# Dave-he/unet-watermark

Hardware: AMD Instinct MI355X
Metric: train_images_per_sec (higher is better)
Workload: dtype f32 storage and accumulation; the convolution products of the encoder and decoder layers (3x3, 7x7 stem, stride-2 and 1x1 layers: forward, data gradients, and the weight gradients of the stride-1 3x3 layers and the stem) as fp16x3 splits - every fp32 operand = two fp16 halves (22 mantissa bits), a*b; 1 GPU; Unet-resnet34 512x512 bs16/GPU train step: fwd + Dice + bwd + Adam (BASELINE.json configs[1]); global_batch=16, parallelism=dp1, grad_allreduce=none

## Files before the change

include/uwm.h:

```cpp
#ifndef UWM_H
#define UWM_H
#include <stddef.h>
#include <stdint.h>

#ifdef __cplusplus
extern "C" {
#endif

typedef struct uwm_model* uwm_handle;
typedef void* uwm_stream;

enum { UWM_ENC_RESNET18 = 18, UWM_ENC_RESNET34 = 34, UWM_ENC_RESNET50 = 50,
       UWM_ENC_EFFICIENTNET_B0 = 100, UWM_ENC_EFFICIENTNET_B1 = 101, UWM_ENC_EFFICIENTNET_B2 = 102,
       UWM_ENC_EFFICIENTNET_B3 = 103, UWM_ENC_EFFICIENTNET_B4 = 104, UWM_ENC_EFFICIENTNET_B5 = 105,
       UWM_ENC_EFFICIENTNET_B6 = 106, UWM_ENC_EFFICIENTNET_B7 = 107 };
enum { UWM_ARCH_UNET = 0, UWM_ARCH_UNETPLUSPLUS = 1 };
enum { UWM_T_F32 = 0, UWM_T_I64 = 1, UWM_T_U8 = 2, UWM_T_I32 = 3 };
enum { UWM_KIND_CONV_W = 0, UWM_KIND_BIAS = 1, UWM_KIND_BN_GAMMA = 2, UWM_KIND_BN_BETA = 3,
       UWM_KIND_BN_MEAN = 4, UWM_KIND_BN_VAR = 5 };
enum { UWM_ARENA_PARAM = 0, UWM_ARENA_BUFFER = 1 };
enum { UWM_PREC_F32 = 0, UWM_PREC_BF16X3 = 1, UWM_PREC_BF16X3_ALL = 2, UWM_PREC_F16X3 = 3, UWM_PREC_F16X3_ALL = 4,
       UWM_PREC_F16X1 = 5, UWM_PREC_F16X3_BWD2 = 6 };

typedef struct {
// ... 356 lines not shown
int    uwm_op_morph(const uint8_t* in, uint8_t* out, int N, int H, int W, int dilate, int shape, int kw, int kh,
                    int iterations, void* workspace, size_t workspace_bytes, uwm_stream stream);
int    uwm_op_components(const uint8_t* in, int32_t* labels ,
                         int32_t* areas , int N, int H, int W,
                         void* workspace, size_t workspace_bytes, uwm_stream stream);

int  uwm_set_side_stream(uwm_handle h, int on);

int  uwm_prof_enable(int on);
int  uwm_prof_collect(double* out, int max_classes);
const char* uwm_prof_class_name(int cls);

int  uwm_debug_lookup(uwm_handle h, const char* key, long long* offset, long long* count);

typedef struct {
  const float* ptr; const float* scale; const float* shift;
  int C, H, W, up, relu;
} uwm_src;
int  uwm_op_preprocess_u8_nhwc4(const uint8_t* images, long long npix, int C, const float* mean, const float* std, float* out,
                                uwm_stream stream);
int  uwm_op_set_igemm_f16x3(int on);
int  uwm_op_conv(const uwm_src* s0, const uwm_src* s1, const float* w, int wrows, int Kpad, int kh, int kw, int stride,
                 int pad, int N, int Cout, const float* bias, float* y, double* stats, int cfg, uwm_stream stream);
int  uwm_op_dgrad(const float* dy, int N, int Ho, int Wo, int Cout, const float* wd, int Cin, int KpadD, int kh, int kw,
                  int stride, int pad, int H, int W, const float* addend, const float* mask, const float* mscale,
                  const float* mshift, float* dx, uwm_stream stream);
int  uwm_op_set_f16x3_products(int n);
int  uwm_op_dgrad_f16x3(const float* dy, int N, int H, int W, int Cout, int CoutP, const float* w, int Kpad, int Cin,
                        const float* addend, const float* mask, const float* mscale, const float* mshift, const float* bnb_mean,
                        const float* bnb_rstd, const float* bnb_y, double* sums, int nrep, long long sums_stride, float* dx, int cfg,
                        uwm_stream stream);
int  uwm_op_wgrad(const uwm_src* s0, const uwm_src* s1, const float* dy, int N, int Ho, int Wo, int Cout, int wrows,
                  int Kpad, int kh, int kw, int stride, int pad, float* dw, int force_igemm, uwm_stream stream);
int  uwm_op_pack_dgrad(const float* w, int Cout, int Kpad, int ntaps, int Cin, float* wd, int KpadD, int CoutP,
                       uwm_stream stream);
int  uwm_op_maxpool(const uwm_src* in, int N, float* out, uint8_t* idx, uwm_stream stream);
int  uwm_op_maxpool_backward(const float* gout, const uint8_t* idx, const float* addend, const uwm_src* in, int N,
                             float* gin, uwm_stream stream);
int  uwm_op_bn_backward(const float* g, const float* y, const float* mean, const float* rstd, const float* gamma,
                        double* scratch2c, float* dy, float* dgamma, float* dbeta, long long npix, int C, uwm_stream stream);
int  uwm_op_bn_backward_act(const float* g, const float* y, const float* mean, const float* rstd, const float* gamma,
                            const float* scale, const float* shift, const float* se_s, const float* gpool, int N, long long hw,
                            int C, double* scratch2c, float* dy, float* dgamma, float* dbeta, float* xmax, uwm_stream stream);
int  uwm_op_dgrad_upsplit(const float* dy, int N, int H, int W, int Cout, const float* wd, int C0, int C1, int KpadD,
                          float* gprev, const float* pmask, const float* pscale, const float* pshift, float* gskip,
                          uwm_stream stream);
int  uwm_op_upsplit(const float* dcat, int N, int H, int W, int C0, int C1, float* gprev, const float* pmask,
                    const float* pscale, const float* pshift, float* gskip, uwm_stream stream);
int  uwm_op_residual(const float* y, const float* s2, const float* b2, const float* id, const float* sd, const float* bd,
                     float* out, long long npix, int C, uwm_stream stream);

#ifdef __cplusplus
}
#endif
#endif
```

unet-watermark_amd/_lib.py:

```python
from __future__ import annotations

import ctypes as C
import os
import subprocess
import sys
from pathlib import Path

os.environ.setdefault("GPU_MAX_HW_QUEUES", "8")

_PKG_DIR = Path(__file__).resolve().parent
_CSRC = _PKG_DIR / "csrc"
LIB_PATH = _PKG_DIR / "libuwm.so"
SOURCES = ["uwm_route.hip", "conv_igemm.hip", "conv_patch.hip", "conv_patch16.hip", "conv_wino.hip", "conv_wino8.hip", "conv_wino_x3.hip", "conv_f16x3.hip", "conv_f16x3v2.hip", "conv_stem_f16x3.hip", "conv_up2.hip", "conv_up2_f16.hip", "conv_c16_f16.hip", "conv_gemm.hip", "conv_head.hip", "mbconv.hip", "wgrad_igemm.hip", "wgrad_patch.hip", "wgrad_wino.hip", "wgrad_f16x3.hip", "wgrad_c16.hip", "wgrad_gemm.hip", "wgrad_stem.hip", "elementwise.hip", "loss.hip", "loss_ext.hip", "mask_post.hip", "mask_score.hip", "mask_dist.hip", "mask_enhance.hip", "resize_u8.hip", "tile_u8.hip", "tta.hip", "pair_mask_u8.hip", "synth_u8.hip", "synth_text_u8.hip", "extract_u8.hip", "text_enhance.hip", "filter_u8.hip", "augment_u8.hip", "augment_ext_u8.hip", "jpeg_u8.hip", "jpeg_ragged_u8.hip", "uwm_model.hip"]
HIP_ARCH = "gfx950"
EXTRA_FLAGS = {name: ["-Xclang", "-target-feature", "-Xclang", "-packed-fp32-ops"]
               for name in ("conv_f16x3.hip", "conv_f16x3v2.hip", "wgrad_f16x3.hip", "conv_stem_f16x3.hip")}
EXTRA_FLAGS["synth_u8.hip"] = ["-ffp-contract=off"]
EXTRA_FLAGS["synth_text_u8.hip"] = ["-ffp-contract=off"]
EXTRA_FLAGS["extract_u8.hip"] = ["-ffp-contract=off"]
EXTRA_FLAGS["text_enhance.hip"] = ["-ffp-contract=off"]


class uwm_unet_desc(C.Structure):
    _fields_ = [("encoder", C.c_int), ("in_channels", C.c_int), ("classes", C.c_int),
# ... 139 lines not shown
    "uwm_resize_threshold": (I, [P, I, I, I, I, I, I, F, I, P, P, P]),
    "uwm_mask_element": (I, [I, I, I, P]),
    "uwm_mask_workspace_bytes": (Z, [I, I, I]),
    "uwm_optimize_mask": (I, [P, P, I, I, I, I, P, P, Z, P]),
    "uwm_mask_ragged_workspace_bytes": (Z, [I, Z, L]),
    "uwm_optimize_masks_ragged": (I, [P, P, Z, P, I, I, L, L, P, P, Z, P]),
    "uwm_score_masks_workspace_bytes": (Z, [I, Z, L]),
    "uwm_score_masks_ragged": (I, [P, P, Z, P, P, I, L, L, P, P, Z, P]),
    "uwm_edt_workspace_bytes": (Z, [I, Z, L]),
    "uwm_edt_ragged": (I, [P, Z, P, I, L, L, P, P, Z, P]),
    "uwm_surface_distances_workspace_bytes": (Z, [I, Z, L]),
    "uwm_surface_distances_ragged": (I, [P, P, Z, P, I, L, L, P, P, P, Z, P]),
    "uwm_enhance_masks_workspace_bytes": (Z, [I, Z]),
    "uwm_enhance_masks_ragged": (I, [P, P, Z, P, I, I, I, I, L, P, P, Z, P]),
    "uwm_enhance_gauss_taps": (I, [I, C.POINTER(C.c_float)]),
    "uwm_text_enhance_workspace_bytes": (Z, [L, I]),
    "uwm_text_enhance_ragged": (I, [P, P, Z, P, I, I, L, L, P, Z, P, P, Z, P]),
    "uwm_extract_workspace_bytes": (Z, [I, L, I]),
    "uwm_extract_regions_ragged": (I, [P, Z, P, P, Z, P, I, I, I, I, L, L, P, Z, P, P, P, P, Z, P]),
    "uwm_extract_cutouts_ragged": (I, [P, Z, P, P, Z, P, I, P, I, L, P, Z, P, P, Z, P]),
    "uwm_op_morph": (I, [P, P, I, I, I, I, I, I, I, I, P, Z, P]),
    "uwm_op_components": (I, [P, P, P, I, I, I, P, Z, P]),
    "uwm_set_side_stream": (I, [P, I]),
    "uwm_prof_enable": (I, [I]),
    "uwm_prof_collect": (I, [C.POINTER(C.c_double), I]),
    "uwm_prof_class_name": (C.c_char_p, [I]),
    "uwm_debug_lookup": (I, [P, C.c_char_p, C.POINTER(L), C.POINTER(L)]),
    "uwm_op_set_igemm_f16x3": (I, [I]),
    "uwm_op_conv": (I, [C.POINTER(uwm_src), C.POINTER(uwm_src), P, I, I, I, I, I, I, I, I, P, P, P, I, P]),
    "uwm_op_dgrad": (I, [P, I, I, I, I, P, I, I, I, I, I, I, I, I, P, P, P, P, P, P]),
    "uwm_op_set_f16x3_products": (I, [I]),
    "uwm_op_dgrad_f16x3": (I, [P, I, I, I, I, I, P, I, I, P, P, P, P, P, P, P, P, I, L, P, I, P]),
    "uwm_op_wgrad": (I, [C.POINTER(uwm_src), C.POINTER(uwm_src), P, I, I, I, I, I, I, I, I, I, I, P, I, P]),
    "uwm_op_pack_dgrad": (I, [P, I, I, I, I, P, I, I, P]),
    "uwm_op_maxpool": (I, [C.POINTER(uwm_src), I, P, P, P]),
    "uwm_op_maxpool_backward": (I, [P, P, P, C.POINTER(uwm_src), I, P, P]),
    "uwm_op_bn_backward": (I, [P, P, P, P, P, P, P, P, P, L, I, P]),
    "uwm_op_bn_backward_act": (I, [P, P, P, P, P, P, P, P, P, I, L, I, P, P, P, P, P, P]),
    "uwm_op_dgrad_upsplit": (I, [P, I, I, I, I, P, I, I, I, P, P, P, P, P, P]),
    "uwm_op_upsplit": (I, [P, I, I, I, I, I, P, P, P, P, P, P]),
    "uwm_op_residual": (I, [P, P, P, P, P, P, P, L, I, P]),
}

_lib = None


def build_library(force: bool = False, verbose: bool = False) -> Path:
    srcs = [_CSRC / s for s in SOURCES]
    hdrs = [_CSRC / "uwm_kernels.h", _PKG_DIR.parent / "include" / "uwm.h"] + sorted(_CSRC.glob("*.inc"))
    if LIB_PATH.exists() and not force:
        newest = max(p.stat().st_mtime for p in srcs + hdrs)
        if LIB_PATH.stat().st_mtime >= newest:
            return LIB_PATH
    hipcc = os.environ.get("HIPCC", "/opt/rocm/bin/hipcc")
    objdir = _PKG_DIR / "build"
    objdir.mkdir(exist_ok=True)
    procs = []
    hdr_m = max(p.stat().st_mtime for p in hdrs + [Path(__file__)])
    for s in srcs:
        o = objdir / (s.stem + ".o")
        if not force and o.exists() and o.stat().st_mtime >= max(s.stat().st_mtime, hdr_m):
            procs.append((None, None, o))
            continue
        cmd = [hipcc, f"--offload-arch={HIP_ARCH}", "-O3", "-std=c++17", "-fPIC"] + EXTRA_FLAGS.get(s.name, []) + ["-c", str(s), "-o", str(o)]
        procs.append((cmd, subprocess.Popen(cmd, stdout=subprocess.PIPE, stderr=subprocess.STDOUT), o))
    objs = []
# ... 81 lines not shown
```

unet-watermark_amd/csrc/uwm_abi.inc:

```
extern "C" {

const char* uwm_last_error(void) { return g_err; }
int uwm_version(void) { return 1; }

int uwm_create(const uwm_unet_desc* desc, uwm_handle* out) {
  if (!desc || !out) return fail("uwm_create: null argument");
  uwm_model* m = new uwm_model();
  m->desc = *desc;
  if (m->desc.bn_eps <= 0.f) m->desc.bn_eps = 1e-5f;
  if (m->desc.bn_momentum <= 0.f) m->desc.bn_momentum = 0.1f;
  if (build_model(m)) { delete m; return 1; }
  const char* e = getenv("UWM_SIDE_STREAM");
  m->use_side = e ? atoi(e) : 1;
  if (const char* pe = getenv("UWM_PRECISION")) {
    static const char* names[7] = {"f32", "bf16x3", "bf16x3_all", "f16x3", "f16x3_all", "f16x1", "f16x3_bwd2"};
    int found = -1;
    for (int i = 0; i < 7; ++i) if (!strcmp(pe, names[i]) || (pe[0] == '0' + i && !pe[1])) found = i;
    if (found < 0) { delete m; return fail("uwm_create: UWM_PRECISION=%s is not a precision mode (f32 | bf16x3 | bf16x3_all | f16x3 | f16x3_all | f16x1 | f16x3_bwd2 or 0..6)", pe); }
    m->prec = found; m->plan.prec = found; m->prec_from_env = found != UWM_PREC_F32;
  }
  if (const char* pf = getenv("UWM_F16X3_MIN_WGS")) m->f3_min_wgs = atoi(pf) > 0 ? atoi(pf) : 0;
  m->wino_mode = winograd_mode();
  m->plan.wino_mode = m->wino_mode;
  *out = m; return 0;
// ... 1570 lines not shown
int uwm_op_dgrad_upsplit(const float* dy, int N, int H, int W, int Cout, const float* wd, int C0, int C1, int KpadD,
                         float* gprev, const float* pmask, const float* pscale, const float* pshift, float* gskip,
                         uwm_stream stream) {
  if (!dy || !wd || !gprev || (C1 > 0 && !gskip)) return fail("uwm_op_dgrad_upsplit: null argument");
  ConvArgs a; memset(&a, 0, sizeof(a));
  a.s0 = mk_src(dy, Cout, H, W); a.s1 = a.s0; a.C0 = Cout; a.Ctot = Cout;
  a.w = wd; a.wrows = C0 + C1; a.Kpad = KpadD; a.ntaps = 9; a.kw = 3;
  a.N = N; a.Ho = H; a.Wo = W; a.Cout = C0 + C1; a.M = N * H * W;
  a.Hl = H; a.Wl = W; a.smul = 1; a.rmul = -1; a.off = 1; a.sdiv = 1;
  a.out = gskip; a.out_up = gprev; a.up_c0 = C0; a.up_mask = pmask; a.up_mscale = pscale; a.up_mshift = pshift;
  a.dv_ctot = make_fastdiv(a.Ctot); a.dv_kw = make_fastdiv(a.kw);
  if (!op_wino_shape(a, 3, 3, 1, 1) || (H & 1) || (W & 1)) return fail("uwm_op_dgrad_upsplit: needs even H >= 8, W >= 16, channels %% 8 == 0");
  if (g_op_ig16) {
    static float* xm = nullptr;
    if (!xm) HIPCHK(hipMalloc((void**)&xm, 32 * sizeof(float)));
    LCHK(launch_absmax32(dy, (size_t)N * H * W * Cout, xm, (hipStream_t)stream));
    a.ig16 = 1; a.xmax = xm;
  }
  if (op_wino_prepare(a, 1, (hipStream_t)stream)) return 1;
  LCHK(launch_conv(a, (hipStream_t)stream));
  return 0;
}
int uwm_op_wgrad(const uwm_src* s0, const uwm_src* s1, const float* dy, int N, int Ho, int Wo, int Cout, int wrows, int Kpad,
                 int kh, int kw, int stride, int pad, float* dw, int force_igemm, uwm_stream stream) {
  if (!s0 || !dy || !dw) return fail("uwm_op_wgrad: null argument");
  WgradArgs a; memset(&a, 0, sizeof(a));
  a.s0 = to_src(s0); a.C0 = a.s0.C;
  if (s1) { a.s1 = to_src(s1); a.Ctot = a.C0 + a.s1.C; } else { a.s1 = a.s0; a.Ctot = a.C0; }
  a.dy = dy; a.dw = dw; a.wrows = wrows; a.Kpad = Kpad; a.ntaps = kh * kw; a.kw = kw;
  a.N = N; a.Ho = Ho; a.Wo = Wo; a.Cout = Cout; a.M = N * Ho * Wo;
  a.Hl = a.s0.H << a.s0.up; a.Wl = a.s0.W << a.s0.up; a.stride = stride; a.pad = pad;
  a.dv_ctot = make_fastdiv(a.Ctot); a.dv_kw = make_fastdiv(a.kw);
  a.force_igemm = force_igemm;
  if ((force_igemm & 0xff) == 6 || (force_igemm & 0xff) == 7) {
    static float* xm = nullptr;
    if (!xm) HIPCHK(hipMalloc((void**)&xm, 32 * sizeof(float)));
    LCHK(launch_absmax32(dy, (size_t)N * Ho * Wo * Cout, xm, (hipStream_t)stream));
    a.prec = 2; a.nprod = g_op_f3_nprod; a.xmax = xm;
  }
  LCHK(launch_wgrad(a, (hipStream_t)stream));
  return 0;
}
int uwm_op_pack_dgrad(const float* w, int Cout, int Kpad, int ntaps, int Cin, float* wd, int KpadD, int CoutP,
                      uwm_stream stream) {
  if (!w || !wd) return fail("uwm_op_pack_dgrad: null argument");
  LCHK(launch_pack_dgrad(w, Cout, Kpad, ntaps, Cin, wd, KpadD, CoutP, (hipStream_t)stream));
  return 0;
}
int uwm_op_bn_backward(const float* g, const float* y, const float* mean, const float* rstd, const float* gamma,
                       double* scratch2c, float* dy, float* dgamma, float* dbeta, long long npix, int C, uwm_stream stream) {
  if (!g || !y || !mean || !rstd || !gamma || !scratch2c || !dy || !dgamma || !dbeta || npix < 1) return fail("uwm_op_bn_backward: bad argument");
  hipStream_t st = (hipStream_t)stream;
  HIPCHK(hipMemsetAsync(scratch2c, 0, 2 * (size_t)C * sizeof(double), st));
  LCHK(launch_bn_bwd_reduce(g, y, mean, rstd, scratch2c, scratch2c + C, (size_t)npix, C, st));
  LCHK(launch_bn_bwd_apply(g, y, mean, rstd, gamma, scratch2c, scratch2c + C, dy, dgamma, dbeta, (size_t)npix, C, st));
  return 0;
}
int uwm_op_bn_backward_act(const float* g, const float* y, const float* mean, const float* rstd, const float* gamma,
                           const float* scale, const float* shift, const float* se_s, const float* gpool, int N, long long hw,
                           int C, double* scratch2c, float* dy, float* dgamma, float* dbeta, float* xmax, uwm_stream stream) {
  if (!g || !y || !mean || !rstd || !gamma || !scale || !shift || !scratch2c || !dy || !dgamma || !dbeta || N < 1 || hw < 1 ||
      C < 4 || (C & 3) || (!se_s != !gpool))
    return fail("uwm_op_bn_backward_act: bad argument");
  hipStream_t st = (hipStream_t)stream;
  HIPCHK(hipMemsetAsync(scratch2c, 0, 2 * (size_t)C * sizeof(double), st));
  if (xmax) HIPCHK(hipMemsetAsync(xmax, 0, 32 * sizeof(float), st));
  LCHK(launch_bn_bwd_act(g, y, mean, rstd, gamma, scale, shift, se_s, gpool, N, (size_t)hw, scratch2c, scratch2c + C, dy, dgamma,
                         dbeta, C, st, xmax));
  return 0;
}
int uwm_op_upsplit(const float* dcat, int N, int H, int W, int C0, int C1, float* gprev, const float* pmask,
                   const float* pscale, const float* pshift, float* gskip, uwm_stream stream) {
  if (!dcat || !gprev) return fail("uwm_op_upsplit: null argument");
  LCHK(launch_upsplit(dcat, N, H, W, C0, C1, gprev, pmask, pscale, pshift, gskip, (hipStream_t)stream));
  return 0;
// ... 76 lines not shown
```

unet-watermark_amd/csrc/uwm_kernels.h:

```cpp
#pragma once
#include <hip/hip_runtime.h>
#include <hip/hip_ext.h>
#include <stdint.h>
#include <stddef.h>
#include <atomic>

struct uwm_loss_spec;

namespace uwm {

struct Src {
  const float* ptr;
  const float* scale;
  const float* shift;
  int C, H, W;
  int up;
  int relu;
};

struct FastDiv {
  unsigned mg, d;
};
static inline FastDiv make_fastdiv(unsigned d) {
  FastDiv f; f.d = d; f.mg = (d <= 1) ? 0u : (unsigned)((0x100000000ull / d) + 1ull); return f;
// ... 160 lines not shown
      hipExtLaunchKernelGGL(kernel, grid, block, lds, st, e0_, e1_, 0, __VA_ARGS__);                         \
    } else {                                                                                                 \
      hipLaunchKernelGGL(kernel, grid, block, lds, st, __VA_ARGS__);                                         \
    }                                                                                                        \
  } while (0)
int  prof_collect(double* out );
const char* prof_class_name(int cls);

enum ConvKernel { kConvInvalid = 0, kConvUp2, kConvUp2F16, kConvUp2Dgrad, kConvUp2DgradF16, kConvC16F16, kConvC32F16, kConvGemm, kConvHead,
                  kConvHeadDgrad, kConvF16x3, kConvF16x3v2, kConvWinoX3, kConvWino, kConvWino8, kConvPatch16, kConvPatch, kConvS2Dgrad, kConvIgemm };
struct ConvRoute { ConvKernel k; int v; };
ConvRoute conv_route(const ConvArgs& a, int force_cfg);
hipError_t launch_conv(const ConvArgs& a, hipStream_t st, int force_cfg = -1);
bool conv_epilogue_carries_bnb(const ConvArgs& a);
enum WgradKernel { kWgradInvalid = 0, kWgradGemm, kWgradUp2, kWgradF16x3, kWgradStem, kWgradC16, kWgradWino, kWgradPatch, kWgradIgemm };
struct WgradRoute { WgradKernel k; int v; };
WgradRoute wgrad_route(const WgradArgs& a);
hipError_t launch_wgrad(const WgradArgs& a, hipStream_t st);
hipError_t launch_conv_igemm(const ConvArgs& a, hipStream_t st, int cfg);
bool conv_s2_dgrad_applicable(const ConvArgs& a);
hipError_t launch_conv_s2_dgrad(const ConvArgs& a, hipStream_t st, int cfg);
hipError_t launch_wgrad_igemm(const WgradArgs& a, hipStream_t st, bool f16);
bool wgrad_patch_applicable(const WgradArgs& a);
hipError_t launch_wgrad_patch(const WgradArgs& a, hipStream_t st);
bool wgrad_wino_applicable(const WgradArgs& a);
hipError_t launch_wgrad_wino(const WgradArgs& a, hipStream_t st);
size_t wgrad_wino_scratch_floats();
float* wgrad_op_scratch();
bool wgrad_c16_applicable(const WgradArgs& a);
hipError_t launch_wgrad_c16(const WgradArgs& a, hipStream_t st);
hipError_t launch_wgrad_reduce(const float* part, int nsplit, size_t n4, float* dw, hipStream_t st, ReduceQueue* rq = nullptr);
hipError_t launch_wgrad_reduce_multi(ReduceQueue& q, hipStream_t st);
bool wgrad_f16x3_applicable(const WgradArgs& a);
hipError_t launch_wgrad_f16x3(const WgradArgs& a, hipStream_t st);
bool wgrad_stem_applicable(const WgradArgs& a);
hipError_t launch_wgrad_stem(const WgradArgs& a, hipStream_t st);
bool wgrad_gemm_applicable(const WgradArgs& a);
hipError_t launch_wgrad_gemm(const WgradArgs& a, hipStream_t st);
bool wgrad_gemm_preferred(const WgradArgs& a);
bool wgrad_up2_applicable(const WgradArgs& a);
hipError_t launch_wgrad_up2(const WgradArgs& a, hipStream_t st);
bool conv_gemm_applicable(const ConvArgs& a);
hipError_t launch_conv_gemm(const ConvArgs& a, hipStream_t st, int bn);
bool conv_gemm_preferred(const ConvArgs& a);
bool conv_up2_applicable(const ConvArgs& a);
hipError_t launch_conv_up2(const ConvArgs& a, hipStream_t st);
bool conv_up2_dgrad_applicable(const ConvArgs& a);
hipError_t launch_conv_up2_dgrad(const ConvArgs& a, hipStream_t st);
hipError_t launch_conv_up2_f16(const ConvArgs& a, hipStream_t st);
hipError_t launch_conv_up2_dgrad_f16(const ConvArgs& a, hipStream_t st);
bool conv_c16_f16_applicable(const ConvArgs& a);
hipError_t launch_conv_c16_f16(const ConvArgs& a, hipStream_t st);
bool conv_c32_f16_applicable(const ConvArgs& a);
hipError_t launch_conv_c32_f16(const ConvArgs& a, hipStream_t st);
bool wgrad_up2_f16_shape(const WgradArgs& a);
int wgrad_up2_f16_parts(const WgradArgs& a);
hipError_t launch_wgrad_up2_f16(const WgradArgs& a, hipStream_t st);
bool conv_patch_applicable(const ConvArgs& a);
bool conv_patch16_applicable(const ConvArgs& a);
hipError_t launch_conv_patch16(const ConvArgs& a, hipStream_t st);
hipError_t launch_conv_patch(const ConvArgs& a, hipStream_t st, int bn);
bool conv_wino_applicable(const ConvArgs& a);
hipError_t launch_conv_wino(const ConvArgs& a, hipStream_t st, int bn = 0);
bool conv_head_applicable(const ConvArgs& a);
hipError_t launch_conv_head(const ConvArgs& a, hipStream_t st);
bool conv_head_dgrad_applicable(const ConvArgs& a);
hipError_t launch_conv_head_dgrad(const ConvArgs& a, hipStream_t st);
// ... 340 lines not shown
```

unet-watermark_amd/csrc/uwm_route.hip:

```cpp
#include "uwm_kernels.h"
#include <stdio.h>
#include <stdlib.h>

namespace uwm {

static int g_winograd = -1;
bool winograd_enabled() {
  if (g_winograd < 0) { const char* e = getenv("UWM_WINOGRAD"); g_winograd = (e && e[0] == '0') ? 0 : 1; }
  return g_winograd != 0;
}
void winograd_set_mode(int mode) { g_winograd = mode; }
int winograd_mode() { (void)winograd_enabled(); return g_winograd; }
int device_cu_count() {
  static int cus[64] = {0};
  int dev = 0; (void)hipGetDevice(&dev);
  if (dev < 0 || dev >= 64) return 256;
  if (!cus[dev] && (hipDeviceGetAttribute(&cus[dev], hipDeviceAttributeMultiprocessorCount, dev) != hipSuccess || cus[dev] <= 0)) cus[dev] = 256;
  return cus[dev];
}

struct RouteSwitches {
  bool trace = dbg_flag("UWM_TRACE_CONV");
  bool no_up2 = dbg_flag("UWM_NO_UP2"), no_up2_wgrad = dbg_flag("UWM_NO_UP2_WGRAD"), no_head = dbg_flag("UWM_NO_CONV_HEAD");
  bool no_bnb_y = dbg_flag("UWM_NO_BNB_Y"), no_igemm_bnb = dbg_flag("UWM_NO_IGEMM_BNB");
  bool no_narrow_1x1 = dbg_flag("UWM_NO_NARROW_1X1"), no_wgrad_ig16 = dbg_flag("UWM_NO_WGRAD_IG16");
};
static const RouteSwitches& switches() { static const RouteSwitches s; return s; }

struct ConvCaps { bool bnb, bnb_y, out_up, bnb_out_up; };
static ConvCaps conv_caps(ConvKernel k) {
  switch (k) {
    case kConvWino:         return {true, true, true, true};
    case kConvWinoX3:       return {true, false, true, true};
    case kConvF16x3:        return {true, true, true, false};
    case kConvUp2Dgrad: case kConvUp2DgradF16: return {true, false, true, true};
    case kConvF16x3v2: case kConvGemm: case kConvS2Dgrad: case kConvIgemm: return {true, true, false, false};
    case kConvC16F16: case kConvC32F16: case kConvPatch16: case kConvHeadDgrad: return {true, false, false, false};
    default:                return {false, false, false, false};
  }
}
ConvRoute conv_route(const ConvArgs& a, int cfg) {
  const RouteSwitches& sw = switches();
  const bool aut = cfg < 0;
  const ConvRoute invalid = {kConvInvalid, 0};
  auto wino = [&](int bn) -> ConvRoute {
    if (bn == 8 || (bn <= 0 && !a.bnb_mean && !a.bnb_y && !a.out_up && conv_wino8_applicable(a))) return {kConvWino8, 0};
    return {kConvWino, bn};
  };
  auto up2 = [&]() -> ConvRoute { return {a.ig16 ? kConvUp2F16 : kConvUp2, 0}; };
  if (cfg == 700) return up2();
  if (cfg == 710 || (aut && a.ig16 && a.prec != 2 && conv_c16_f16_applicable(a))) return {kConvC16F16, 0};
  if (cfg == 711 || (aut && a.ig16 && a.prec != 2 && conv_c32_f16_applicable(a))) return {kConvC32F16, 0};
  if (cfg >= 800 && cfg < 1000) return {kConvGemm, cfg - 800};
  if (cfg == 500) return {kConvHead, 0};
  if ((cfg >= 600 && cfg <= 607) || (aut && a.prec == 2)) {
    const int v = aut ? 0 : cfg - 600;
    if (a.wu_layout == 1) return (v == 4 || v == 6 || !conv_f16x3v2_applicable(a)) ? invalid : ConvRoute{kConvF16x3v2, v == 5};
    return (v >= 4 || !conv_f16x3_applicable(a)) ? invalid : ConvRoute{kConvF16x3, v};
// ... 63 lines not shown
                     !(a.out_up ? a.up_mask : (a.bnb_y ? a.bnb_y : a.mask)) || a.up_accum))
    return hipErrorInvalidValue;
  if (a.out_up && (!c.out_up || ((a.Ho | a.Wo) & 1) || (a.up_c0 & 3) || a.up_c0 > a.Cout || a.addend || a.mask || a.bias || a.bnb_y ||
                   (a.ssum && !a.bnb_mean) || (a.up_c0 < a.Cout && !a.out)))
    return hipErrorInvalidValue;
  switch (r.k) {
    case kConvUp2:         return launch_conv_up2(a, st);
    case kConvUp2F16:      return launch_conv_up2_f16(a, st);
    case kConvUp2Dgrad:    return launch_conv_up2_dgrad(a, st);
    case kConvUp2DgradF16: return launch_conv_up2_dgrad_f16(a, st);
    case kConvC16F16:      return launch_conv_c16_f16(a, st);
    case kConvC32F16:      return launch_conv_c32_f16(a, st);
    case kConvGemm:        return launch_conv_gemm(a, st, r.v);
    case kConvHead:        return launch_conv_head(a, st);
    case kConvHeadDgrad:   return launch_conv_head_dgrad(a, st);
    case kConvF16x3:       return launch_conv_f16x3(a, st, r.v);
    case kConvF16x3v2:     return launch_conv_f16x3v2(a, st, r.v != 0);
    case kConvWinoX3:      return launch_conv_wino_x3(a, st);
    case kConvWino:        return launch_conv_wino(a, st, r.v);
    case kConvWino8:       return launch_conv_wino8(a, st);
    case kConvPatch16:     return launch_conv_patch16(a, st);
    case kConvPatch:       return launch_conv_patch(a, st, r.v);
    case kConvS2Dgrad:     return launch_conv_s2_dgrad(a, st, r.v);
    case kConvIgemm:       return launch_conv_igemm(a, st, r.v);
    default:               return hipErrorInvalidValue;
  }
}

WgradRoute wgrad_route(const WgradArgs& a) {
  const RouteSwitches& sw = switches();
  const int f = a.force_igemm & 0xff;
  const bool aut = f == 0, no_up2 = sw.no_up2 || sw.no_up2_wgrad;
  if (f == 4) return {kWgradGemm, 0};
  if (a.prec == 2 && (aut || f == 6)) {
    if (a.xmax && !no_up2 && wgrad_up2_applicable(a) && wgrad_up2_f16_shape(a)) return {kWgradUp2, 0};
    if (wgrad_f16x3_applicable(a)) return {kWgradF16x3, 0};
  }
  if (f == 6) {
    if (a.prec == 2 && wgrad_stem_applicable(a)) return {kWgradStem, 0};
    if (a.prec == 2 && a.Cout == 16 && wgrad_c16_applicable(a)) return {kWgradC16, 0};
    return {kWgradInvalid, 0};
  }
  if (aut && !no_up2 && wgrad_up2_applicable(a)) return {kWgradUp2, 0};
  if (aut && wgrad_stem_applicable(a)) return {kWgradStem, 0};
  if (aut && wgrad_gemm_preferred(a)) return {kWgradGemm, 0};
  if (aut && wgrad_c16_applicable(a)) return {kWgradC16, 0};
  if (aut && wino_mode_of(a.wino) != 0 && wgrad_wino_applicable(a)) return {kWgradWino, 0};
  if (f != 1 && f != 7 && wgrad_patch_applicable(a)) return {kWgradPatch, 0};
  const bool f16 = !sw.no_wgrad_ig16 && a.prec == 2 && a.xmax && (aut || f == 7) && (a.Ctot & 31) == 0 && (a.Cout & 31) == 0;
  return {kWgradIgemm, f16 ? 1 : 0};
}

hipError_t launch_wgrad(const WgradArgs& a, hipStream_t st) {
  if (switches().trace)
    fprintf(stderr, "wgrad N=%d Ctot=%d(C0=%d) Cout=%d wrows=%d Ho=%d Wo=%d Hl=%d Wl=%d taps=%d stride=%d wino=%d patch=%d gflop=%.2f\n", a.N, a.Ctot,
            a.C0, a.Cout, a.wrows, a.Ho, a.Wo, a.Hl, a.Wl, a.ntaps, a.stride, (int)(wino_mode_of(a.wino) != 0 && wgrad_wino_applicable(a)),
            (int)wgrad_patch_applicable(a), a.flops * 1e-9);
  const WgradRoute r = wgrad_route(a);
  switch (r.k) {
    case kWgradGemm:  return launch_wgrad_gemm(a, st);
    case kWgradUp2:   return launch_wgrad_up2(a, st);
    case kWgradF16x3: return launch_wgrad_f16x3(a, st);
    case kWgradStem:  return launch_wgrad_stem(a, st);
    case kWgradC16:   return launch_wgrad_c16(a, st);
    case kWgradWino:  return launch_wgrad_wino(a, st);
    case kWgradPatch: return launch_wgrad_patch(a, st);
    case kWgradIgemm: return launch_wgrad_igemm(a, st, r.v != 0);
    default:          return hipErrorInvalidValue;
  }
}

}
```

unet-watermark_amd/csrc/wgrad_f16x3.hip:

```cpp
#include "uwm_kernels.h"

namespace uwm {

typedef float f4 __attribute__((ext_vector_type(4)));
typedef _Float16 h8 __attribute__((ext_vector_type(8)));
typedef _Float16 h4 __attribute__((ext_vector_type(4)));

#ifndef UWM_WG16_ABL
#define UWM_WG16_ABL 0
#endif
#ifndef UWM_WG16_XCD
#define UWM_WG16_XCD 1
#endif
template <int WX> struct WG16 {
  static constexpr int kWR = 128 / WX, kWX = WX, kWPW = WX + 2, kWPH = kWR + 2;
  static constexpr int kWXB = kWPH * kWPW * 136;
  static constexpr int kWStage = 32768 + ((kWXB + 255) & ~255);
  static constexpr int kWXRounds = (kWPH * kWPW * 8 + 511) / 512;
};
constexpr int kWDyB = 128 * 256;
constexpr int kWXS = 136;
constexpr int kWLT = 512;
constexpr int kWDyRounds = 128 * 16 / kWLT;

// ... 164 lines not shown
          if (UWM_WG16_ABL & 1) { if (it < 9) { acc[0][it][0] += (float)xh[it % 3][0] + (float)xl[it % 3][1]; acc[1][it][1] += (float)ah[1][2] + (float)al[0][3]; } continue; }
          const int pt = it - 1, ps = (it + 2) % 3, cs = it % 3;
          if (it < 9) acc[0][it] = __builtin_amdgcn_mfma_f32_16x16x32_f16(ah[0], xh[cs], acc[0][it], 0, 0, 0);
          if (NP >= 2 && it >= 1) acc[0][pt] = __builtin_amdgcn_mfma_f32_16x16x32_f16(ah[0], xl[ps], acc[0][pt], 0, 0, 0);
          if (it < 9) acc[1][it] = __builtin_amdgcn_mfma_f32_16x16x32_f16(ah[1], xh[cs], acc[1][it], 0, 0, 0);
          if (NP >= 2 && it >= 1) acc[1][pt] = __builtin_amdgcn_mfma_f32_16x16x32_f16(ah[1], xl[ps], acc[1][pt], 0, 0, 0);
          if (NP >= 3 && it >= 1) acc[0][pt] = __builtin_amdgcn_mfma_f32_16x16x32_f16(al[0], xh[ps], acc[0][pt], 0, 0, 0);
          if (NP >= 3 && it >= 1) acc[1][pt] = __builtin_amdgcn_mfma_f32_16x16x32_f16(al[1], xh[ps], acc[1][pt], 0, 0, 0);
          __builtin_amdgcn_sched_barrier(0);
        }
      }
      __syncthreads();
    }
    const float ixs = 1.f / xs;
    float* const dst = a.nsplit > 1 ? a.part + (size_t)split * a.wrows * a.Kpad : a.dw;
    const int ci = b0 + 16 * bf + (lane & 15);
#pragma unroll
    for (int cf = 0; cf < 2; ++cf)
#pragma unroll
      for (int t = 0; t < 9; ++t)
#pragma unroll
        for (int e = 0; e < 4; ++e) {
          const int row = a0 + 16 * (2 * cp + cf) + 4 * (lane >> 4) + e;
          if (row < a.wrows && ci < a.Ctot) {
            float* pd = dst + (size_t)row * a.Kpad + t * a.Ctot + ci;
            const float v = acc[cf][t][e] * ixs;
            if (UWM_WG16_ABL & 8) { if (v == 123.456f) *pd = v; }
            else if (a.nsplit > 1) *pd = v; else *pd += v;
          }
        }
  }
}

static int wgrad_f16x3_wx(const WgradArgs& a) {
  if ((a.Wo % 32) == 0 && (a.Ho % 4) == 0) return 32;
  if ((a.Wo % 16) == 0 && (a.Ho % 8) == 0) return 16;
  return 0;
}
bool wgrad_f16x3_applicable(const WgradArgs& a) {
  return a.xmax != nullptr && a.ntaps == 9 && a.kw == 3 && a.stride == 1 && a.pad == 1 && (a.Ctot & 31) == 0 && (a.C0 & 31) == 0 &&
         (a.Cout & 3) == 0 && a.wrows <= a.Cout && a.Kpad == 9 * a.Ctot && a.Hl == a.Ho && a.Wl == a.Wo &&
         wgrad_f16x3_wx(a) != 0 && (a.s0.C & 3) == 0 && (a.s1.C & 3) == 0 && a.Wo < 256 * 128 &&
         (size_t)a.N * a.s0.H * a.s0.W < (1ull << 31) && (size_t)a.N * a.s1.H * a.s1.W < (1ull << 31) && (size_t)8 * a.Wo * a.Cout < (1ull << 31);
}

template <int WX, int NP>
static hipError_t launch_wg16p(WgradArgs& a, hipStream_t st, int pairs, int sps, int nstages) {
  const size_t lds = (size_t)2 * WG16<WX>::kWStage;
  static DevOnce lds_attr;
  { hipError_t e = lds_attr.set_max_lds((const void*)wgrad_f16x3_kernel<WX, NP>, lds); if (e != hipSuccess) return e; }
  UWM_LAUNCH(43, a.flops, a.bytes, (wgrad_f16x3_kernel<WX, NP>), dim3((unsigned)(pairs * a.nsplit)), dim3(768), lds, st, a, sps, nstages);
  return hipGetLastError();
}
template <int WX>
static hipError_t launch_wg16(WgradArgs& a, hipStream_t st, int pairs, int sps, int nstages) {
  const int np = (a.nprod >= 1 && a.nprod <= 3) ? a.nprod : 3;
  return np == 3 ? launch_wg16p<WX, 3>(a, st, pairs, sps, nstages) : np == 2 ? launch_wg16p<WX, 2>(a, st, pairs, sps, nstages) : launch_wg16p<WX, 1>(a, st, pairs, sps, nstages);
}

hipError_t launch_wgrad_f16x3(const WgradArgs& a0, hipStream_t st) {
  WgradArgs a = a0;
  if (!wgrad_f16x3_applicable(a)) return hipErrorInvalidValue;
  const int wx = wgrad_f16x3_wx(a);
  const int pairs = ((a.wrows + 63) / 64) * (a.Ctot / 32);
  const int nstages = a.N * (a.Ho / (128 / wx)) * (a.Wo / wx);
  static const int cu_cap = dbg_int("UWM_WG16_CUS", 0);
  const int cus = cu_cap > 0 ? cu_cap : (a.cu_share > 0 ? device_cu_count() * a.cu_share / 4 : device_cu_count());
  int nsplit = (cus + pairs - 1) / pairs;
  if (nsplit > nstages / 4) nsplit = nstages / 4;
  if (nsplit < 1) nsplit = 1;
  const size_t image = (size_t)a.wrows * a.Kpad;
  if (nsplit > 1 && (!a.part || a.part_floats < 2 * image)) { a.part = wgrad_op_scratch(); a.part_floats = wgrad_wino_scratch_floats(); a.rq = nullptr; }
  if (nsplit > 1 && (!a.part || (size_t)nsplit * image > a.part_floats)) nsplit = a.part ? (int)(a.part_floats / image) : 1;
  if (nsplit < 1) nsplit = 1;
  const int sps = (nstages + nsplit - 1) / nsplit;
  nsplit = (nstages + sps - 1) / sps;
  a.nsplit = nsplit; a.msplit = sps;
  hipError_t e = wx == 32 ? launch_wg16<32>(a, st, pairs, sps, nstages) : launch_wg16<16>(a, st, pairs, sps, nstages);
  if (e != hipSuccess) return e;
  if (nsplit > 1) return launch_wgrad_reduce(a.part, nsplit, image / 4, a.dw, st, a.rq);
  return hipSuccess;
}

}
```

Baseline: 1197 images/s.

## Add rows32 f16x3 wgrad kernel for layers with at most 32 output rows

Adds a specialised fp16x3 weight-gradient kernel for stride-1 3x3 layers whose weight row count is at most 32 (e.g. decoder layers with Cout=16 or 32). Each block tiles 32 output rows by 64 input channels instead of 64 by 32, so no MFMA work is spent on padded rows. It uses a smaller dy LDS stage with its own swizzle. The router picks it automatically when applicable, and an env switch can disable it; a last-kernel query is also exposed for debugging. The tile has fewer blocks per layer, which leans more on the split-K reduction, and the new LDS layout and indexing carry correctness risk.

```diff
diff --git a/include/uwm.h b/include/uwm.h
--- a/include/uwm.h
+++ b/include/uwm.h
@@ -412,6 +412,7 @@
                         uwm_stream stream);
 int  uwm_op_wgrad(const uwm_src* s0, const uwm_src* s1, const float* dy, int N, int Ho, int Wo, int Cout, int wrows,
                   int Kpad, int kh, int kw, int stride, int pad, float* dw, int force_igemm, uwm_stream stream);
+const char* uwm_op_last_kernel(void);
 int  uwm_op_pack_dgrad(const float* w, int Cout, int Kpad, int ntaps, int Cin, float* wd, int KpadD, int CoutP,
                        uwm_stream stream);
 int  uwm_op_maxpool(const uwm_src* in, int N, float* out, uint8_t* idx, uwm_stream stream);
diff --git a/unet-watermark_amd/_lib.py b/unet-watermark_amd/_lib.py
--- a/unet-watermark_amd/_lib.py
+++ b/unet-watermark_amd/_lib.py
@@ -195,6 +195,7 @@
     "uwm_op_set_f16x3_products": (I, [I]),
     "uwm_op_dgrad_f16x3": (I, [P, I, I, I, I, I, P, I, I, P, P, P, P, P, P, P, P, I, L, P, I, P]),
     "uwm_op_wgrad": (I, [C.POINTER(uwm_src), C.POINTER(uwm_src), P, I, I, I, I, I, I, I, I, I, I, P, I, P]),
+    "uwm_op_last_kernel": (C.c_char_p, []),
     "uwm_op_pack_dgrad": (I, [P, I, I, I, I, P, I, I, P]),
     "uwm_op_maxpool": (I, [C.POINTER(uwm_src), I, P, P, P]),
     "uwm_op_maxpool_backward": (I, [P, P, P, C.POINTER(uwm_src), I, P, P]),
diff --git a/unet-watermark_amd/csrc/uwm_abi.inc b/unet-watermark_amd/csrc/uwm_abi.inc
--- a/unet-watermark_amd/csrc/uwm_abi.inc
+++ b/unet-watermark_amd/csrc/uwm_abi.inc
@@ -1626,7 +1626,7 @@
   a.Hl = a.s0.H << a.s0.up; a.Wl = a.s0.W << a.s0.up; a.stride = stride; a.pad = pad;
   a.dv_ctot = make_fastdiv(a.Ctot); a.dv_kw = make_fastdiv(a.kw);
   a.force_igemm = force_igemm;
-  if ((force_igemm & 0xff) == 6 || (force_igemm & 0xff) == 7) {
+  if ((force_igemm & 0xff) == 6 || (force_igemm & 0xff) == 7 || (force_igemm & 0xff) == 8) {
     static float* xm = nullptr;
     if (!xm) HIPCHK(hipMalloc((void**)&xm, 32 * sizeof(float)));
     LCHK(launch_absmax32(dy, (size_t)N * Ho * Wo * Cout, xm, (hipStream_t)stream));
@@ -1635,6 +1635,7 @@
   LCHK(launch_wgrad(a, (hipStream_t)stream));
   return 0;
 }
+const char* uwm_op_last_kernel(void) { return route_last(); }
 int uwm_op_pack_dgrad(const float* w, int Cout, int Kpad, int ntaps, int Cin, float* wd, int KpadD, int CoutP,
                       uwm_stream stream) {
   if (!w || !wd) return fail("uwm_op_pack_dgrad: null argument");
diff --git a/unet-watermark_amd/csrc/uwm_kernels.h b/unet-watermark_amd/csrc/uwm_kernels.h
--- a/unet-watermark_amd/csrc/uwm_kernels.h
+++ b/unet-watermark_amd/csrc/uwm_kernels.h
@@ -216,7 +216,8 @@
 hipError_t launch_wgrad_reduce(const float* part, int nsplit, size_t n4, float* dw, hipStream_t st, ReduceQueue* rq = nullptr);
 hipError_t launch_wgrad_reduce_multi(ReduceQueue& q, hipStream_t st);
 bool wgrad_f16x3_applicable(const WgradArgs& a);
-hipError_t launch_wgrad_f16x3(const WgradArgs& a, hipStream_t st);
+bool wgrad_f16x3_rows32_applicable(const WgradArgs& a);
+hipError_t launch_wgrad_f16x3(const WgradArgs& a, hipStream_t st, bool rows32 = false);
 bool wgrad_stem_applicable(const WgradArgs& a);
 hipError_t launch_wgrad_stem(const WgradArgs& a, hipStream_t st);
 bool wgrad_gemm_applicable(const WgradArgs& a);
diff --git a/unet-watermark_amd/csrc/uwm_route.hip b/unet-watermark_amd/csrc/uwm_route.hip
--- a/unet-watermark_amd/csrc/uwm_route.hip
+++ b/unet-watermark_amd/csrc/uwm_route.hip
@@ -24,6 +24,7 @@
   bool no_up2 = dbg_flag("UWM_NO_UP2"), no_up2_wgrad = dbg_flag("UWM_NO_UP2_WGRAD"), no_head = dbg_flag("UWM_NO_CONV_HEAD");
   bool no_bnb_y = dbg_flag("UWM_NO_BNB_Y"), no_igemm_bnb = dbg_flag("UWM_NO_IGEMM_BNB");
   bool no_narrow_1x1 = dbg_flag("UWM_NO_NARROW_1X1"), no_wgrad_ig16 = dbg_flag("UWM_NO_WGRAD_IG16");
+  bool no_wgrad_rows32 = dbg_flag("UWM_NO_WGRAD_ROWS32");
 };
 static const RouteSwitches& switches() { static const RouteSwitches s; return s; }
 
@@ -153,11 +154,12 @@
   const int f = a.force_igemm & 0xff;
   const bool aut = f == 0, no_up2 = sw.no_up2 || sw.no_up2_wgrad;
   if (f == 4) return {kWgradGemm, 0};
-  if (a.prec == 2 && (aut || f == 6)) {
+  if (a.prec == 2 && (aut || f == 6 || f == 8)) {
     if (a.xmax && !no_up2 && wgrad_up2_applicable(a) && wgrad_up2_f16_shape(a)) return {kWgradUp2, 0};
-    if (wgrad_f16x3_applicable(a)) return {kWgradF16x3, 0};
+    if (wgrad_f16x3_applicable(a))
+      return {kWgradF16x3, f != 6 && !sw.no_wgrad_rows32 && wgrad_f16x3_rows32_applicable(a) ? 1 : 0};
   }
-  if (f == 6) {
+  if (f == 6 || f == 8) {
     if (a.prec == 2 && wgrad_stem_applicable(a)) return {kWgradStem, 0};
     if (a.prec == 2 && a.Cout == 16 && wgrad_c16_applicable(a)) return {kWgradC16, 0};
     return {kWgradInvalid, 0};
@@ -181,7 +183,7 @@
   switch (r.k) {
     case kWgradGemm:  return launch_wgrad_gemm(a, st);
     case kWgradUp2:   return launch_wgrad_up2(a, st);
-    case kWgradF16x3: return launch_wgrad_f16x3(a, st);
+    case kWgradF16x3: return launch_wgrad_f16x3(a, st, r.v != 0);
     case kWgradStem:  return launch_wgrad_stem(a, st);
     case kWgradC16:   return launch_wgrad_c16(a, st);
     case kWgradWino:  return launch_wgrad_wino(a, st);
diff --git a/unet-watermark_amd/csrc/wgrad_f16x3.hip b/unet-watermark_amd/csrc/wgrad_f16x3.hip
--- a/unet-watermark_amd/csrc/wgrad_f16x3.hip
+++ b/unet-watermark_amd/csrc/wgrad_f16x3.hip
@@ -220,6 +220,200 @@
   }
 }
 
+constexpr int kRXS = 272;
+constexpr int kRDyB = 128 * 128;
+constexpr int kRXB = 6 * 34 * kRXS;
+constexpr int kRStage = kRDyB + ((kRXB + 255) & ~255);
+constexpr int kRDyRounds = 128 * 8 / kWLT;
+constexpr int kRXRounds = (6 * 34 * 16 + kWLT - 1) / kWLT;
+
+__device__ __forceinline__ int off_dy32(int row, int ch) { return 128 * row + 16 * (ch ^ (((row >> 1) & 1) << 1) ^ (((row >> 3) & 1) << 2)); }
+
+template <int NP = 3>
+__global__ __launch_bounds__(768, 1) void wgrad_f16x3_rows32_kernel(const WgradArgs a, int stages_per_split, int nstages) {
+  constexpr int kWR = 4, kWX = 32, kWPW = 34, kWPH = 6, kKS = 4;
+  extern __shared__ __attribute__((aligned(256))) char wsm[];
+  const int tid = threadIdx.x, lane = tid & 63, wave = __builtin_amdgcn_readfirstlane(tid >> 6);
+  const bool is_mma = wave < 4;
+  const int ltid = tid - 256;
+
+  const int pairs = a.Ctot / 64;
+  const int lin = (int)uwm_xcd_tile();
+  const int split = lin / pairs, tb = lin - split * pairs;
+  const int b0 = tb * 64;
+  const int st0 = split * stages_per_split, st1 = min(nstages, st0 + stages_per_split);
+  const int tilesX = a.Wo / kWX, tilesY = a.Ho / kWR;
+
+  float xs = 1.f;
+  if (a.xmax) xs = uwm_dy_scale(a.xmax);
+
+  f4 acc[2][9];
+#pragma unroll
+  for (int cf = 0; cf < 2; ++cf)
+#pragma unroll
+    for (int t = 0; t < 9; ++t) acc[cf][t] = (f4){0.f, 0.f, 0.f, 0.f};
+
+  if (!is_mma) {
+    const bool first = b0 < a.C0;
+    const Src& s = first ? a.s0 : a.s1;
+    const int cl = first ? b0 : b0 - a.C0;
+    const int dcu = ltid & 7;
+    const bool dok = dcu * 4 < a.Cout;
+    const int xcu = ltid & 15;
+    f4 xsc = {1.f, 1.f, 1.f, 1.f}, xsh = {0.f, 0.f, 0.f, 0.f};
+    const bool xhas = s.scale != nullptr;
+    if (xhas) { xsc = *(const f4*)(s.scale + cl + xcu * 4); xsh = *(const f4*)(s.shift + cl + xcu * 4); }
+    const int xrelu = s.relu;
+    struct Stage { f4 dv[kRDyRounds]; f4 xv[kRXRounds]; unsigned xok; };
+    int dgo[kRDyRounds], dlo[kRDyRounds], xpy[kRXRounds], xlo[kRXRounds];
+#pragma unroll
+    for (int rd = 0; rd < kRDyRounds; ++rd) {
+      const int px = (rd * kWLT + ltid) >> 3;
+      dgo[rd] = ((px / kWX) * a.Wo + (px % kWX)) * a.Cout;
+      dlo[rd] = off_dy32(px, dcu >> 1) + (dcu & 1) * 8;
+    }
+#pragma unroll
+    for (int rd = 0; rd < kRXRounds; ++rd) {
+      const int pp = (rd * kWLT + ltid) >> 4;
+      const bool act = pp < kWPH * kWPW;
+      const int py = act ? pp / kWPW : 0, px = act ? pp - py * kWPW : 0;
+      xpy[rd] = act ? ((py << 8) | px) : -1;
+      xlo[rd] = pp * kRXS + ((xcu >> 1) & 1) * 64 + (xcu >> 2) * 16 + (xcu & 1) * 8;
+    }
+    const float* const dyp = a.dy + dcu * 4;
+    const float* const xp = s.ptr + cl + xcu * 4;
+    auto stage_load = [&](int st, Stage& sg) {
+      int q = st;
+      const int tx = q % tilesX; q /= tilesX;
+      const int ty = q % tilesY; const int n = q / tilesY;
+      const int y0 = ty * kWR, x0 = tx * kWX;
+      const float* const dbase = dyp + (((size_t)n * a.Ho + y0) * a.Wo + x0) * a.Cout;
+#pragma unroll
+      for (int rd = 0; rd < kRDyRounds; ++rd) sg.dv[rd] = dok ? *(const f4*)(dbase + dgo[rd]) : (f4){0.f, 0.f, 0.f, 0.f};
+      sg.xok = 0;
+      const int nb = n * s.H;
+#pragma unroll
+      for (int rd = 0; rd < kRXRounds; ++rd) {
+        const int hl = y0 - 1 + (xpy[rd] >> 8), wl = x0 - 1 + (xpy[rd] & 255);
+        const bool ok = xpy[rd] >= 0 && hl >= 0 && hl < a.Hl && wl >= 0 && wl < a.Wl;
+        const int hc = min(max(hl, 0), a.Hl - 1), wc = min(max(wl, 0), a.Wl - 1);
+        sg.xv[rd] = *(const f4*)(xp + (size_t)(((nb + (hc >> s.up)) * s.W + (wc >> s.up))) * s.C);
+        sg.xok |= (ok ? 1u : 0u) << rd;
+      }
+    };
+    auto split_store = [&](char* dst_hi, char* dst_lo, f4 v, bool clamp) {
+      h4 hi, lo;
+#pragma unroll
+      for (int e = 0; e < 4; ++e) {
+        const float x = clamp ? uwm_clamp_h(v[e]) : v[e];
+        const _Float16 h = (_Float16)x;
+        hi[e] = h; lo[e] = (_Float16)(x - (float)h);
+      }
+      *(h4*)dst_hi = hi; *(h4*)dst_lo = lo;
+    };
+    auto stage_store = [&](int buf, const Stage& sg) {
+      char* const dyb = wsm + buf * kRStage;
+      char* const xb = dyb + kRDyB;
+#pragma unroll
+      for (int rd = 0; rd < kRDyRounds; ++rd) split_store(dyb + dlo[rd], dyb + (dlo[rd] ^ 64), sg.dv[rd] * xs, false);
+#pragma unroll
+      for (int rd = 0; rd < kRXRounds; ++rd) {
+        if (xpy[rd] >= 0) {
+          f4 v = sg.xv[rd];
+          if (xhas) {
+            v = v * xsc + xsh;
+            if (xrelu) { v.x = fmaxf(v.x, 0.f); v.y = fmaxf(v.y, 0.f); v.z = fmaxf(v.z, 0.f); v.w = fmaxf(v.w, 0.f); }
+          }
+          if (!((sg.xok >> rd) & 1u)) v = (f4){0.f, 0.f, 0.f, 0.f};
+          split_store(xb + xlo[rd], xb + xlo[rd] + 128, v, true);
+        }
+      }
+    };
+    Stage sA, sB;
+    const int ns = st1 - st0;
+    if (ns > 0) {
+      stage_load(st0, sA);
+      stage_load(ns > 1 ? st0 + 1 : st0, sB);
+      stage_store(0, sA);
+    }
+    __syncthreads();
+    for (int i = 0; i < ns; i += 2) {
+      {
+        if (i + 1 < ns) stage_store(1, sB);
+        stage_load(st0 + (i + 2 < ns ? i + 2 : ns - 1), sA);
+        __syncthreads();
+      }
+      if (i + 1 < ns) {
+        if (i + 2 < ns) stage_store(0, sA);
+        stage_load(st0 + (i + 3 < ns ? i + 3 : ns - 1), sB);
+        __syncthreads();
+      }
+    }
+  } else {
+    const int bf = wave;
+    const int kg = lane >> 4, q = (lane & 15) >> 2, p = lane & 3;
+    int dyo[2][2];
+#pragma unroll
+    for (int cf = 0; cf < 2; ++cf)
+#pragma unroll
+      for (int rdx = 0; rdx < 2; ++rdx)
+        dyo[cf][rdx] = off_dy32(8 * kg + 4 * rdx + q, 2 * cf + (p >> 1)) + 8 * (p & 1);
+    const int xo = (8 * kg + q) * kRXS + (p >> 1) * 64 + bf * 16 + 8 * (p & 1);
+    const int ns = st1 - st0;
+    __syncthreads();
+    for (int i = 0; i < ns; ++i) {
+      const char* const dyb = wsm + (i & 1) * kRStage;
+      const char* const xb = dyb + kRDyB;
+#pragma unroll
+      for (int kr = 0; kr < kKS; ++kr) {
+        h8 ah[2], al[2];
+#pragma unroll
+        for (int cf = 0; cf < 2; ++cf) {
+          ah[cf] = uwm_tr_pair(dyb + kr * 32 * 128, dyo[cf][0], dyo[cf][1]);
+          al[cf] = uwm_tr_pair(dyb + kr * 32 * 128, dyo[cf][0] ^ 64, dyo[cf][1] ^ 64);
+        }
+        h8 xh[3], xl[3];
+        auto x_read = [&](int t) {
+          const int r = t / 3, sx = t % 3;
+          const char* xp = xb + ((kr + r) * kWPW + sx) * kRXS + xo;
+          xh[t % 3] = uwm_tr_pair(xp, 0, 4 * kRXS);
+          xl[t % 3] = uwm_tr_pair(xp, 128, 4 * kRXS + 128);
+        };
+        x_read(0);
+#pragma unroll
+        for (int it = 0; it < 10; ++it) {
+          if (it + 1 < 9) x_read(it + 1);
+          const int pt = it - 1, ps = (it + 2) % 3, cs = it % 3;
+          if (it < 9) acc[0][it] = __builtin_amdgcn_mfma_f32_16x16x32_f16(ah[0], xh[cs], acc[0][it], 0, 0, 0);
+          if (NP >= 2 && it >= 1) acc[0][pt] = __builtin_amdgcn_mfma_f32_16x16x32_f16(ah[0], xl[ps], acc[0][pt], 0, 0, 0);
+          if (it < 9) acc[1][it] = __builtin_amdgcn_mfma_f32_16x16x32_f16(ah[1], xh[cs], acc[1][it], 0, 0, 0);
+          if (NP >= 2 && it >= 1) acc[1][pt] = __builtin_amdgcn_mfma_f32_16x16x32_f16(ah[1], xl[ps], acc[1][pt], 0, 0, 0);
+          if (NP >= 3 && it >= 1) acc[0][pt] = __builtin_amdgcn_mfma_f32_16x16x32_f16(al[0], xh[ps], acc[0][pt], 0, 0, 0);
+          if (NP >= 3 && it >= 1) acc[1][pt] = __builtin_amdgcn_mfma_f32_16x16x32_f16(al[1], xh[ps], acc[1][pt], 0, 0, 0);
+          __builtin_amdgcn_sched_barrier(0);
+        }
+      }
+      __syncthreads();
+    }
+    const float ixs = 1.f / xs;
+    float* const dst = a.nsplit > 1 ? a.part + (size_t)split * a.wrows * a.Kpad : a.dw;
+    const int ci = b0 + 16 * bf + (lane & 15);
+#pragma unroll
+    for (int cf = 0; cf < 2; ++cf)
+#pragma unroll
+      for (int t = 0; t < 9; ++t)
+#pragma unroll
+        for (int e = 0; e < 4; ++e) {
+          const int row = 16 * cf + 4 * (lane >> 4) + e;
+          if (row < a.wrows && ci < a.Ctot) {
+            float* pd = dst + (size_t)row * a.Kpad + t * a.Ctot + ci;
+            const float v = acc[cf][t][e] * ixs;
+            if (a.nsplit > 1) *pd = v; else *pd += v;
+          }
+        }
+  }
+}
+
 static int wgrad_f16x3_wx(const WgradArgs& a) {
   if ((a.Wo % 32) == 0 && (a.Ho % 4) == 0) return 32;
   if ((a.Wo % 16) == 0 && (a.Ho % 8) == 0) return 16;
@@ -230,6 +424,10 @@
          (a.Cout & 3) == 0 && a.wrows <= a.Cout && a.Kpad == 9 * a.Ctot && a.Hl == a.Ho && a.Wl == a.Wo &&
          wgrad_f16x3_wx(a) != 0 && (a.s0.C & 3) == 0 && (a.s1.C & 3) == 0 && a.Wo < 256 * 128 &&
          (size_t)a.N * a.s0.H * a.s0.W < (1ull << 31) && (size_t)a.N * a.s1.H * a.s1.W < (1ull << 31) && (size_t)8 * a.Wo * a.Cout < (1ull << 31);
+}
+
+bool wgrad_f16x3_rows32_applicable(const WgradArgs& a) {
+  return wgrad_f16x3_applicable(a) && a.wrows <= 32 && (a.Ctot & 63) == 0 && (a.C0 & 63) == 0 && wgrad_f16x3_wx(a) == 32;
 }
 
 template <int WX, int NP>
@@ -246,11 +444,24 @@
   return np == 3 ? launch_wg16p<WX, 3>(a, st, pairs, sps, nstages) : np == 2 ? launch_wg16p<WX, 2>(a, st, pairs, sps, nstages) : launch_wg16p<WX, 1>(a, st, pairs, sps, nstages);
 }
 
-hipError_t launch_wgrad_f16x3(const WgradArgs& a0, hipStream_t st) {
+template <int NP>
+static hipError_t launch_wg16r32p(WgradArgs& a, hipStream_t st, int pairs, int sps, int nstages) {
+  const size_t lds = (size_t)2 * kRStage;
+  static DevOnce lds_attr;
+  { hipError_t e = lds_attr.set_max_lds((const void*)wgrad_f16x3_rows32_kernel<NP>, lds); if (e != hipSuccess) return e; }
+  UWM_LAUNCH(43, a.flops, a.bytes, (wgrad_f16x3_rows32_kernel<NP>), dim3((unsigned)(pairs * a.nsplit)), dim3(768), lds, st, a, sps, nstages);
+  return hipGetLastError();
+}
+static hipError_t launch_wg16r32(WgradArgs& a, hipStream_t st, int pairs, int sps, int nstages) {
+  const int np = (a.nprod >= 1 && a.nprod <= 3) ? a.nprod : 3;
+  return np == 3 ? launch_wg16r32p<3>(a, st, pairs, sps, nstages) : np == 2 ? launch_wg16r32p<2>(a, st, pairs, sps, nstages) : launch_wg16r32p<1>(a, st, pairs, sps, nstages);
+}
+
+hipError_t launch_wgrad_f16x3(const WgradArgs& a0, hipStream_t st, bool rows32) {
   WgradArgs a = a0;
-  if (!wgrad_f16x3_applicable(a)) return hipErrorInvalidValue;
+  if (!(rows32 ? wgrad_f16x3_rows32_applicable(a) : wgrad_f16x3_applicable(a))) return hipErrorInvalidValue;
   const int wx = wgrad_f16x3_wx(a);
-  const int pairs = ((a.wrows + 63) / 64) * (a.Ctot / 32);
+  const int pairs = rows32 ? a.Ctot / 64 : ((a.wrows + 63) / 64) * (a.Ctot / 32);
   const int nstages = a.N * (a.Ho / (128 / wx)) * (a.Wo / wx);
   static const int cu_cap = dbg_int("UWM_WG16_CUS", 0);
   const int cus = cu_cap > 0 ? cu_cap : (a.cu_share > 0 ? device_cu_count() * a.cu_share / 4 : device_cu_count());
@@ -264,7 +475,7 @@
   const int sps = (nstages + nsplit - 1) / nsplit;
   nsplit = (nstages + sps - 1) / sps;
   a.nsplit = nsplit; a.msplit = sps;
-  hipError_t e = wx == 32 ? launch_wg16<32>(a, st, pairs, sps, nstages) : launch_wg16<16>(a, st, pairs, sps, nstages);
+  hipError_t e = rows32 ? launch_wg16r32(a, st, pairs, sps, nstages) : wx == 32 ? launch_wg16<32>(a, st, pairs, sps, nstages) : launch_wg16<16>(a, st, pairs, sps, nstages);
   if (e != hipSuccess) return e;
   if (nsplit > 1) return launch_wgrad_reduce(a.part, nsplit, image / 4, a.dw, st, a.rq);
   return hipSuccess;
```

Result: no change. 1204 images/s, median of 6 (+0.6%).
